# iKrishneel/fcn_object_detector

Measured on AMD Instinct MI355X. Metric: frames/sec forward 448x448 @1 GPU; train imgs/sec @1/2/4/8 GPUs, higher is better.
Workload: dtype f32; 1 GPU; configs[1]: single-GPU forward, DetectNet GoogLeNet conv stack + coverage/bbox heads (graph of models/deploy.prototxt), batch=1, 448x448, random-init weights; global_batch=1, parallelism=replicas x1, frames_in_flight=4

## Files before the change

fcn_object_detector_amd/engine.py:

```python
from __future__ import annotations

import ctypes as C
import os
import threading
from collections import namedtuple
from dataclasses import dataclass, field
from typing import Callable, Dict, List, Optional, Sequence, Tuple, Union

import numpy as np

from . import lib as L
from . import storage as S
from . import tune as T
from .netspec import Layer, NetSpec, bn_global_stats, crop_window, kernel_stride_pad
from .storage import _r4, _ra, ip_pack_bank, ip_unpack_bank

F32 = np.float32


def graphs_enabled() -> bool:
    return os.environ.get("FCN_NO_GRAPH", "0") in ("", "0")


_replica_ctx = threading.local()
# ... 234 lines not shown
        self.score_acc: Dict[str, DeviceBuffer] = {}
        self.graph_score: Optional[int] = None
        if dtype == "f16" and spec.phase != "TEST":
            raise NotImplementedError("the half-float path is inference only (BASELINE configs[4])")
        self.dtype, self.f16 = dtype, dtype == "f16"
        self.spec = spec
        self.device = device
        self.fuse = fuse
        self.group_convs = group_convs
        self.autotune = autotune
        L.call("fcn_init", device)
        sp = C.c_void_p()
        self.replica = replica if replica is not None else _take_replica_index()
        if self.replica is None:
            L.call("fcn_stream_create", C.byref(sp))
        else:
            L.call("fcn_stream_create_replica", C.byref(sp), int(self.replica))
        self.stream = int(sp.value)
        yes = C.c_int(0)
        L.call("fcn_stream_is_prioritized", self.stream, C.byref(yes))
        self.stream_prioritized = bool(yes.value)
        self.lock = threading.RLock()
        self.shapes = spec.infer(data_shapes)
        self.blobs: Dict[str, Blob] = {}
        self.params_host: Dict[str, List[np.ndarray]] = {}
        self.params_dev: Dict[str, List[DevView]] = {}
        self.ops: List[Op] = []
        self.graph_io: Optional[int] = None
        self.graph_core: Optional[int] = None
        self._staging: Dict[str, DeviceBuffer] = {}
        self._keep: List[object] = []
        self._conv_layer_meta: Dict[str, dict] = {}
        self._group_workspaces: List[DeviceBuffer] = []
        self.aux_dev: Dict[str, DeviceBuffer] = {}
        self._bn_chains: Dict[str, BnChain] = {}
        self._bn_ws_bytes = 0
        self._bn_ws: Optional[DeviceBuffer] = None
        self._lazy_blob_ops: Dict[str, List[Op]] = {}
        self.loss_blobs: Dict[str, float] = {}
        self.device_fed: set = set()
        self.dropout_seed = 0
        self.dropout_index_offset = 0
        self.inputs = spec.data_tops()
        self.outputs = [b for b in spec.output_blobs() if b in self.shapes]
        max_lds = int(tune_max_lds_kb if tune_max_lds_kb is not None else os.environ.get("FCN_TUNE_MAX_LDS_KB", "160")) * 1024
        self.tuner = T.Tuner(self.stream, T.key_suffix(self.shapes.get(self.inputs[0], ()) if self.inputs else None, self.f16, max_lds),
                             spec.phase == "TEST", max_lds, tune_from._chosen_cfgs if tune_from is not None else None)
        self._plan_buffers()
        self._alloc_params(params)
        self._build_ops()
        self.tuner.release()

    @property
    def _chosen_cfgs(self) -> Dict[str, object]:
        return self.tuner.chosen

    def _plan_buffers(self) -> None:
        plan = S.plan_blobs(self.spec, self.shapes, self.inputs, self.outputs, self.f16, self.fuse, os.environ.get("FCN_F16_IMAGE", "1") != "0")
        self.producers, self.consumers = plan.producers, plan.consumers
        self.alias, self.shift, self.copy_concats, self.copy_slices = plan.alias, plan.shift, plan.copy_concats, plan.copy_slices
        self._half_inputs = plan.half_inputs
        bufs = {root: DeviceBuffer(nbytes) for root, nbytes in plan.root_bytes.items()}
        for name, v in plan.views.items():
            b = self.blobs[name] = Blob(name, v.shape)
            b.esize, b.rows, b.is_input = v.esize, v.rows, name in self.inputs
            b.buf, b.coffset, b.cstride = bufs[v.root], v.coffset, v.cstride
# ... 27 lines not shown
        for l in self.spec.param_layers():
            if l.name in self.shared_layers:
                continue
            shapes = self.spec.param_shapes[l.name]
            blobs = params.get(l.name)
            if blobs is None:
                raise KeyError("no parameters for layer %s" % l.name)
            host = []
            for arr, shp in zip(blobs, shapes):
                a = np.ascontiguousarray(arr, dtype=F32)
                if a.shape != tuple(shp):
                    if a.size != int(np.prod(shp)):
                        raise ValueError("layer %s: parameter shape %s does not match %s" % (l.name, a.shape, shp))
                    a = a.reshape(shp)
                host.append(a.copy())
            self.params_host[l.name] = host
        self.param_flat = DeviceBuffer(max(self.param_count, 4) * 4, zero=True)
        for seg in self.param_layout:
            self.param_segs[(seg.layer, seg.index)] = seg
            self.params_dev.setdefault(seg.layer, []).append(DevView(self.param_flat.ptr + 4 * seg.offset, seg.nbytes))
        for l in self.spec.param_layers():
            if l.name not in self.shared_layers:
                self._upload_params(l)

    def _folded_shift(self, l: Layer) -> float:
        return next((sh for t, sh in self._half_inputs.values() if t == l.bottoms[0]), 0.0) if l.type == "Convolution" else 0.0

    def _upload_params(self, l: Layer) -> None:
        if l.name in self.shared_layers:
            raise RuntimeError("layer %s reads the parameters of another engine (share_params): set them there" % l.name)
        packed = [S.pack(self.param_segs[(l.name, i)], h, self._folded_shift(l) if i == 0 else 0.0) for i, h in enumerate(self.params_host[l.name])]
        for arr, dev in zip(packed, self.params_dev[l.name]):
            L.call("fcn_memcpy_h2d_async", dev.ptr, arr.ctypes.data, arr.nbytes, None)
        L.call("fcn_device_sync")

    def set_params(self, layer: str, blobs: Sequence[np.ndarray]) -> None:
        lay = next(l for l in self.spec.layers if l.name == layer)
        if layer in self.shared_layers:
            raise RuntimeError("layer %s reads the parameters of another engine (share_params): set them there" % layer)
        shapes = self.spec.param_shapes[layer]
        self.params_host[layer] = [np.ascontiguousarray(b, dtype=F32).reshape(s).copy() for b, s in zip(blobs, shapes)]
        self._upload_params(lay)

    def read_param(self, layer: str, index: int) -> np.ndarray:
        with self.lock:
            v = self.params_dev[layer][index]
            raw = np.empty(v.nbytes, np.uint8)
            L.call("fcn_memcpy_d2h_async", raw.ctypes.data, v.ptr, raw.nbytes, self.stream)
            L.call("fcn_stream_sync", self.stream)
        return S.unpack(self.param_segs[(layer, index)], raw)

    def _geom(self, l: Layer, ksp: Optional[Tuple[int, int, int]] = None) -> ConvGeom:
        n, cin, h, w = self.blobs[l.bottoms[0]].shape
        _, cout, oh, ow = self.blobs[l.tops[0]].shape
        k, s, pad = ksp or kernel_stride_pad(l.sub("pooling_param" if l.type == "Pooling" else "convolution_param"))
        return ConvGeom(n, cin, h, w, cout, oh, ow, k, s, pad)

    def _conv_groups(self, l: Layer) -> int:
        return int(l.sub("convolution_param").get("group", 1)) if l.type == "Convolution" else 1

    def _conv_desc(self, l: Layer, fused_relu: bool, sig_top: Optional[str], group: int = 0) -> L.ConvDesc:
        g, ng = self._geom(l), self._conv_groups(l)
        xb, yb = self.blobs[l.bottoms[0]], self.blobs[l.tops[0]]
        eps = 16 // xb.esize
        if xb.coffset % eps or xb.cstride % eps:
            raise NotImplementedError("conv input view of %s is not 16-byte aligned" % l.name)
# ... 163 lines not shown
            if t == "InnerProduct":
                relu = self._relu_after(li, l, skip)
                self._conv_layer_meta[l.name] = dict(relu=relu, sigmoid_top=None)
                tasks.append(OpTask(l, self._fwd_inner_product(l, relu), reads=[self._range(l.bottoms[0])], writes=[self._range(l.tops[0])]))
                continue
            if t in ("BatchNorm", "Scale"):
                ch = self._bn_chain_after(li, l, skip)
                tasks.append(OpTask(l, self._fwd_batchnorm(ch), reads=[self._range(ch.x)], writes=[self._range(ch.y)]))
                continue
            if t == "Concat" and l.name not in self.copy_concats:
                continue
            if t == "Slice" and l.name not in self.copy_slices:
                continue
            if t == "Dropout" and spec.phase == "TEST" and (l.tops[0] == l.bottoms[0] or l.tops[0] in self.alias):
                continue
            if t == "Power" and l.tops[0] in self.shift:
                continue
            ops = self._emit_simple(l)
            read = l.bottoms[:1] if t == "Crop" else l.bottoms
            tasks.append(OpTask(l, ops, reads=[self._range(b) for b in read], writes=[self._range(tp) for tp in l.tops],
                                pool_desc=self._fusable_pool_desc(l)))
        return tasks

    def _build_ops(self) -> None:
        tasks = self._collect_tasks()
        if self._bn_ws_bytes:
            self._bn_ws = DeviceBuffer(self._bn_ws_bytes, zero=False)
        if self.fuse and self.spec.phase == "TEST" and os.environ.get("FCN_FUSE_POOL_LRN", "1") != "0":
            tasks = self._fuse_pool_lrn(tasks)
        levels = task_levels(tasks, self.group_convs)
        if self.autotune and self.group_convs and self.fuse and not self.f16 and self.spec.phase == "TEST" and os.environ.get("FCN_LEVEL_MOVE", "1") != "0":
            self.tuner.move_floaters(tasks, levels)
        tail = self._plan_tail(tasks, levels)
        order = sorted(range(len(tasks)), key=lambda i: (levels[i], 1 if isinstance(tasks[i], ConvTask) else 0, i))
        pending: List[ConvTask] = []
        pending_pools: List[OpTask] = []
        cur = None
        for i in order:
            if levels[i] != cur:
                self._emit_convs(pending, pending_pools, tail)
                pending, cur = [], levels[i]
            if tail is not None and any(tasks[i] is ht for ht in tail["heads"]):
                continue
            if isinstance(tasks[i], ConvTask):
                pending.append(tasks[i])
            elif tasks[i].pool_desc is not None and self.fuse and self.group_convs:
                pending_pools.append(tasks[i])
            else:
                self.ops.extend(tasks[i].ops)
        self._emit_convs(pending, pending_pools, tail)
        self.levels = max(levels) + 1 if levels else 0
        if self.score_outputs:
            self._emit_score_ops()

    def _emit_group(self, chunk: List[ConvTask], fused: List[OpTask], tail: Optional[dict]) -> None:
        lib = L.load()
        name = "+".join(it.layer.name for it in chunk)
        flops = sum(it.flops for it in chunk)
        byts = sum(it.bytes for it in chunk)
        arr = (L.ConvDesc * len(chunk))(*[it.desc for it in chunk])
        ws = DeviceBuffer(int(lib.fcn_conv2d_group_workspace_bytes(len(chunk))), zero=False)
        self._group_workspaces.append(ws)
        grp = L.ConvGroup()
        parr = (L.PoolDesc * max(len(fused), 1))(*[pt.pool_desc for pt in fused])
        tune_key = name + ("{+%d pool}" % len(fused) if fused else "")
        tailed = tail is not None and any(id(it) in tail["producers"] for it in chunk)
        if tailed:
            fin = 1 if any(tail["producers"][id(it)] == tail["final_level"] for it in chunk if id(it) in tail["producers"]) else 0
            tail["desc"].finalize = fin
            L.call("fcn_conv2d_group_attach_tail", ws.ptr, C.byref(tail["desc"]))
            tune_key += "{+tail%d}" % fin
            if fin:
                flops += sum(ht.flops for ht in tail["heads"])
                byts += sum(4.0 * ht.desc.Cout * (ht.desc.N * ht.desc.OH * ht.desc.OW + ht.desc.Cin) for ht in tail["heads"])
        cfg = self.tuner.conv_cfg(tune_key, arr, len(chunk), ws, parr, len(fused)) if self.autotune else -1
        L.call("fcn_conv2d_group_prepare_fused", arr, len(chunk), parr, len(fused), ws.ptr, cfg, C.byref(grp))
        self._keep.extend([arr, parr, ws, grp])
        kind = "conv_group" if len(chunk) > 1 else "conv"
        label = "%s [cfg%d %dwg]" % (name, grp.cfg, grp.total_tiles)
        if fused:
            label = "%s {+%s}" % (label, "+".join(pt.layer.name for pt in fused))
            byts += sum(pt.ops[0].bytes for pt in fused)
        if tailed:
            label = "%s {%s %s}" % (label, "tail:" if tail["desc"].finalize else "partial sums of", "+".join(ht.layer.name for ht in tail["heads"]))
        self.ops.append(Op(kind, label, lambda st, g=grp: L.check(lib.fcn_conv2d_fwd_group_f32(C.byref(g), st)), flops, byts))

    def _emit_convs(self, items: List[ConvTask], pools: List[OpTask], tail: Optional[dict]) -> None:
        for base in range(0, len(items), 16):
            chunk = items[base:base + 16]
            fused = pools[:2] if base == 0 and len(chunk) <= 8 else []
            parts = [chunk]
            if self.f16 and self.autotune and not fused and len(chunk) > 1:
                parts = self.tuner.split_level(chunk)
            for part in parts:
                self._emit_group(part, fused, tail)
                fused = []
            if base == 0 and len(chunk) <= 8:
                del pools[:2]
        for pt in pools:
            self.ops.extend(pt.ops)
        pools.clear()

    def _emit_score_ops(self) -> None:
        lib = L.load()
        for nm in self.outputs:
            b = self.blobs[nm]
            if b.esize != 4 or b.lazy_shift:
                raise NotImplementedError("score_outputs: output blob %s is not a plain float32 blob" % nm)
            count = int(np.prod(b.shape)) if b.shape else 1
            acc = DeviceBuffer(max(4 * count, 16), zero=True)
            self.score_acc[nm] = acc
            if b.nchw is not None:
                n, c, h, w = b.nchw
                args = (acc.ptr, b.buf.ptr, n, h * w, c, b.cstride, b.coffset)
            else:
                args = (acc.ptr, b.ptr, 1, 1, count, count, 0)
            self.ops.append(Op("score", "score:" + nm, lambda st, a=args: L.check(lib.fcn_score_accumulate_f32(*a, st)), 0.0, 12.0 * count))

    def _plan_tail(self, tasks: List[Task], levels: List[int]) -> Optional[dict]:
        if self.f16 or self.spec.phase != "TEST" or not (self.fuse and self.group_convs) or os.environ.get("FCN_CONV_TAIL", "0") != "1":
            return None
        conv_idx = [i for i, t in enumerate(tasks) if isinstance(t, ConvTask)]
        if not conv_idx:
            return None
        lh = max(levels[i] for i in conv_idx)
        heads = [i for i in conv_idx if levels[i] == lh]
        if any(levels[i] >= lh for i, t in enumerate(tasks) if not isinstance(t, ConvTask)) or not 1 <= len(heads) <= 4:
            return None
        d0 = tasks[heads[0]].desc
        m = d0.N * d0.OH * d0.OW
        rows = 0
        for i in heads:
            d = tasks[i].desc
            if (d.kh, d.kw, d.stride, d.pad) != (1, 1, 1, 0) or d.x != d0.x or d.x_cstride != d0.x_cstride or d.Cin != d0.Cin or d.Cin % 32 or d.Cin > 1024 or d.Cout % 4 \
# ... 800 lines not shown
            for i, op in enumerate(self.ops):
                acc = []
                for _ in range(reps):
                    for prev in self.ops[:i]:
                        prev.run(self.stream)
                    L.call("fcn_event_record", e0, self.stream)
                    op.run(self.stream)
                    L.call("fcn_event_record", e1, self.stream)
                    L.call("fcn_event_sync", e1)
                    L.call("fcn_event_elapsed_ms", e0, e1, C.byref(ms))
                    acc.append(ms.value)
                out.append((op.kind, op.name, float(np.median(acc)), op.flops, op.bytes))
            L.call("fcn_event_destroy", e0)
            L.call("fcn_event_destroy", e1)
        self.event_pair_floor_ms = floor
        return out

    def close(self) -> None:
        with self.lock:
            lib = L.load()
            for g in (self.graph_io, self.graph_core, self.graph_score):
                if g:
                    lib.fcn_graph_destroy(g)
            self.graph_io = self.graph_core = self.graph_score = None
            if self.stream:
                lib.fcn_stream_sync(self.stream)
                lib.fcn_stream_destroy(self.stream)
                self.stream = 0
            for ws in getattr(self, "_group_workspaces", []):
                if ws.ptr:
                    lib.fcn_conv2d_group_release(ws.ptr)
                    ws.free()
            self._group_workspaces = []
            self.ops = []
            self.tuner.release()

    def __del__(self):
        try:
            self.close()
        except Exception:
            pass


class ForwardPipeline:

    def __init__(self, make_spec: Callable[[], NetSpec], params: Optional[Dict[str, List[np.ndarray]]] = None, device: int = 0, depth: int = 4,
                 max_lds_kb: Optional[int] = 36, **engine_kw):
        if depth < 1:
            raise ValueError("depth must be at least 1")
        self.engines: List[Engine] = []
        if os.environ.get("FCN_PIPE_LDS_KB"):
            max_lds_kb = int(os.environ["FCN_PIPE_LDS_KB"]) or None
        if max_lds_kb is not None:
            engine_kw.setdefault("tune_max_lds_kb", max_lds_kb)
        for i in range(depth):
            self.engines.append(Engine(make_spec(), params=params, device=device, tune_from=self.engines[0] if i else None, replica=i,
                                       **engine_kw))
        self._pending: List[Engine] = []
        self._next = 0

    @property
    def depth(self) -> int:
        return len(self.engines)

    def submit(self, inputs: Dict[str, np.ndarray]) -> None:
        if len(self._pending) >= len(self.engines):
# ... 82 lines not shown
```

fcn_object_detector_amd/lib.py:

```python
from __future__ import annotations

import ctypes as C
import os
import threading
from typing import Optional

_HERE = os.path.dirname(os.path.abspath(__file__))
LIB_PATH = os.environ.get("FCN_LIB_PATH") or os.path.join(_HERE, "libfcnhip.so")


class FcnLibraryError(RuntimeError):
    pass


class FcnError(RuntimeError):
    def __init__(self, code: int, msg: str):
        super().__init__("libfcnhip error %d: %s" % (code, msg))
        self.code = code


class ConvDesc(C.Structure):
    _fields_ = [
        ("x", C.c_void_p), ("w", C.c_void_p), ("bias", C.c_void_p), ("y", C.c_void_p), ("y2", C.c_void_p),
        ("N", C.c_int32), ("H", C.c_int32), ("W", C.c_int32), ("Cin", C.c_int32), ("x_cstride", C.c_int32),
# ... 95 lines not shown
    "fcn_memcpy_h2d_async": (_i, [_vp, _vp, _sz, _vp]),
    "fcn_memcpy_d2h_async": (_i, [_vp, _vp, _sz, _vp]),
    "fcn_memcpy_d2d_async": (_i, [_vp, _vp, _sz, _vp]),
    "fcn_stream_create": (_i, [C.POINTER(_vp)]),
    "fcn_stream_destroy": (_i, [_vp]),
    "fcn_stream_sync": (_i, [_vp]),
    "fcn_event_create": (_i, [C.POINTER(_vp)]),
    "fcn_event_destroy": (_i, [_vp]),
    "fcn_event_record": (_i, [_vp, _vp]),
    "fcn_event_sync": (_i, [_vp]),
    "fcn_event_elapsed_ms": (_i, [_vp, _vp, C.POINTER(_f)]),
    "fcn_graph_begin": (_i, [_vp]),
    "fcn_graph_end": (_i, [_vp, C.POINTER(_vp)]),
    "fcn_graph_launch": (_i, [_vp, _vp]),
    "fcn_graph_destroy": (_i, [_vp]),
    "fcn_stream_create_replica": (_i, [C.POINTER(_vp), _i]),
    "fcn_stream_is_prioritized": (_i, [_vp, C.POINTER(_i)]),
    "fcn_nchw_to_nhwc_f32": (_i, [_vp, _vp, _i, _i, _i, _i, _i, _i, _f, _vp]),
    "fcn_nhwc_to_nchw_f32": (_i, [_vp, _vp, _i, _i, _i, _i, _i, _i, _vp]),
    "fcn_nhwc_to_nchw_multi_f32": (_i, [C.POINTER(LayoutDesc), _i, _vp]),
    "fcn_conv2d_fwd_f32": (_i, [C.POINTER(ConvDesc), _vp]),
    "fcn_conv2d_group_workspace_bytes": (_sz, [_i]),
    "fcn_conv2d_num_configs": (_i, []),
    "fcn_conv2d_first_layer_config": (_i, []),
    "fcn_conv2d_config_lds_bytes": (_i, [_i]),
    "fcn_conv2d_config_waves_k": (_i, [_i]),
    "fcn_conv2d_group_prepare": (_i, [C.POINTER(ConvDesc), _i, _vp, _i, C.POINTER(ConvGroup)]),
    "fcn_conv2d_group_prepare_fused": (_i, [C.POINTER(ConvDesc), _i, C.POINTER(PoolDesc), _i, _vp, _i, C.POINTER(ConvGroup)]),
    "fcn_conv2d_fwd_group_f32": (_i, [C.POINTER(ConvGroup), _vp]),
    "fcn_conv2d_group_release": (_i, [_vp]),
    "fcn_conv2d_tail_scratch_bytes": (C.c_size_t, [C.POINTER(ConvTail)]),
    "fcn_conv2d_tail_arrive_bytes": (C.c_size_t, [C.POINTER(ConvTail)]),
    "fcn_conv2d_group_attach_tail": (_i, [_vp, C.POINTER(ConvTail)]),
    "fcn_maxpool_fwd_f32": (_i, [_vp, _vp, _vp] + [_i] * 12 + [_vp]),
    "fcn_avepool_fwd_f32": (_i, [_vp, _vp] + [_i] * 12 + [_vp]),
    "fcn_lrn_fwd_f32": (_i, [_vp, _vp, _vp, _i, _i, _i, _i, _i, _f, _f, _f, _vp]),
    "fcn_maxpool_lrn5_fwd_f32": (_i, [_vp, _vp] + [_i] * 12 + [_f, _f, _f, _vp]),
    "fcn_maxpool_lrn5_fwd_f16": (_i, [_vp, _vp] + [_i] * 12 + [_f, _f, _f, _vp]),
    "fcn_maxpool_lrn5_conv1x1_fwd_f32": (_i, [_vp] + [_i] * 10 + [_f, _f, _f, _vp, _vp, _i, _i, _vp, _i, _i, _vp]),
    "fcn_maxpool_lrn5_conv1x1_fwd_f16": (_i, [_vp] + [_i] * 10 + [_f, _f, _f, _vp, _vp, _i, _i, _vp, _i, _i, _vp]),
    "fcn_relu_fwd_f32": (_i, [_vp, _vp, _sz, _f, _vp]),
    "fcn_sigmoid_fwd_f32": (_i, [_vp, _vp, _sz, _vp]),
    "fcn_power_fwd_f32": (_i, [_vp, _vp, _sz, _f, _f, _f, _vp]),
    "fcn_eltwise_fwd_f32": (_i, [_vp, _vp, _vp, _sz, _i, _f, _f, _vp]),
    "fcn_copy_channels_f32": (_i, [_vp, _vp, _i, _i, _i, _i, _i, _i, _vp]),
    "fcn_deconv_depthwise_fwd_f32": (_i, [_vp, _vp, _vp, _vp] + [_i] * 12 + [_vp]),
    "fcn_preprocess_bgr8": (_i, [_vp, _i, _i, _vp, _i, _i, _i, _f, _vp, _vp]),
    "fcn_detect_workspace_bytes": (_sz, [C.POINTER(DetectParams), _i]),
    "fcn_detect_decode_group": (_i, [_vp, _vp, _i, _sz, _sz, C.POINTER(DetectParams), _vp, _vp, _vp, _vp, _vp]),
    "fcn_score_masks_workspace_bytes": (_sz, [_i, _i, _i, _i]),
    "fcn_score_masks": (_i, [_vp, _i, _i, _i, _i, _i, _i, _vp, _f, _vp, _i, _i, _vp, _vp, _vp]),
    "fcn_gen_targets": (_i, [_vp, _vp, _vp, _i, _i, _i, _i, _i, _d, _vp, _vp, _vp, _vp, _vp, _vp]),
    "fcn_gen_targets_nhwc": (_i, [_vp, _vp, _vp, _i, _i, _i, _i, _i, _d, _vp, _i, _vp, _vp, _vp, _vp, _i, _vp]),
    "fcn_conv2d_wgrad_workspace_floats": (_sz, [C.POINTER(ConvDesc), C.POINTER(_i)]),
    "fcn_conv2d_wgrad_f32": (_i, [C.POINTER(ConvDesc), _vp, _vp, _vp, _vp]),
    "fcn_conv2d_wgrad_group_workspace_floats": (_sz, [C.POINTER(ConvDesc), _i]),
    "fcn_conv2d_wgrad_group_f32": (_i, [C.POINTER(ConvDesc), _vp, _vp, _i, _vp, _vp]),
    "fcn_conv2d_wgrad_num_configs": (_i, []),
    "fcn_conv2d_wgrad_split_config": (_i, []),
    "fcn_conv2d_wgrad_workspace_floats_cfg": (_sz, [C.POINTER(ConvDesc), _i, C.POINTER(_i)]),
    "fcn_conv2d_wgrad_cfg_f32": (_i, [C.POINTER(ConvDesc), _vp, _vp, _vp, _i, _vp]),
    "fcn_conv2d_wgrad_group_workspace_floats_cfg": (_sz, [C.POINTER(ConvDesc), _i, _i]),
    "fcn_conv2d_wgrad_group_cfg_f32": (_i, [C.POINTER(ConvDesc), _vp, _vp, _i, _vp, _i, _vp]),
    "fcn_conv_weights_flip_f32": (_i, [_vp, _vp, _i, _i, _i, _i, _i, _i, _vp]),
    "fcn_nchw_f32_to_nhwc_f16": (_i, [_vp, _vp, _i, _i, _i, _i, _i, _i, _f, _vp]),
    "fcn_nhwc_f16_to_nchw_f32": (_i, [_vp, _vp, _i, _i, _i, _i, _i, _i, _vp]),
# ... 129 lines not shown
```

fcn_object_detector_amd/tune.py:

```python
from __future__ import annotations

import ctypes as C
import json
import os
from typing import Callable, Dict, Iterable, List, NamedTuple, Optional, Sequence, Tuple

import numpy as np

from . import engine as E
from . import lib as L


def lower_quartile(samples: Sequence[float]) -> float:
    return float(np.percentile(samples, 25))


class Protocol(NamedTuple):
    warm: int
    reps: int
    evict: bool
    samples: int
    stat: Callable[[Sequence[float]], float]
    contenders: int
    margin: float
# ... 164 lines not shown
            op.sel["cfg"] = self.choose(self.key("wgrad:" + "+".join(op.layers)), self._valid_cfg(ncfg),
                                        lambda: self.fastest(range(ncfg), select, lambda: op.run(self.stream), WGRAD)[0])
            op.name += " [cfg%d]" % op.sel["cfg"]

    def split_level(self, chunk: List["E.ConvTask"]) -> List[List["E.ConvTask"]]:
        n = len(chunk)
        if n < 2 or n > 4:
            return [chunk]

        def valid(code) -> bool:
            return isinstance(code, str) and len(code) == n and all(ch.isdigit() and int(ch) < n for ch in code)

        def search() -> str:
            memo: Dict[Tuple[int, ...], float] = {}

            def cost(sub: Tuple[int, ...]) -> float:
                if sub not in memo:
                    memo[sub] = self._subset_ms([chunk[i].desc for i in sub])
                return memo[sub]

            best, best_ms = None, 1e30
            for labels in set_partitions(n):
                ms = sum(cost(tuple(i for i in range(n) if labels[i] == g)) for g in sorted(set(labels)))
                if ms < best_ms - 1e-7:
                    best, best_ms = labels, ms
            return "".join(str(g) for g in best)

        choice = self.choose("cut|" + self.key("+".join(it.layer.name for it in chunk)), valid, search)
        groups: Dict[str, List[E.ConvTask]] = {}
        for it, g in zip(chunk, choice):
            groups.setdefault(g, []).append(it)
        return [groups[g] for g in sorted(groups)]

    def move_floaters(self, tasks: Sequence[object], levels: List[int]) -> None:
        for lv in range(max(levels, default=-1)):
            a_idx, b_idx = ([i for i, t in enumerate(tasks) if levels[i] == l2 and isinstance(t, E.ConvTask)] for l2 in (lv, lv + 1))
            if len(a_idx) < 2 or not b_idx or len(a_idx) > 8:
                continue
            fl = [i for i in a_idx if E.task_floats(tasks, levels, i)]
            if not fl or len(fl) > 3 or len(b_idx) + len(fl) > 8:
                continue

            def valid(code) -> bool:
                return isinstance(code, str) and len(code) == len(fl) and set(code) <= {"0", "1"} and (len(fl) < len(a_idx) or "0" in code)

            def search() -> str:
                pools = {l2: [t.pool_desc for j, t in enumerate(tasks) if levels[j] == l2 and isinstance(t, E.OpTask) and t.pool_desc is not None][:2]
                         for l2 in (lv, lv + 1)}
                memo: Dict[Tuple[int, Tuple[int, ...]], float] = {}

                def cost(l2: int, sub: Tuple[int, ...]) -> float:
                    if (l2, sub) not in memo:
                        memo[(l2, sub)] = min(self._subset_ms([tasks[i].desc for i in sub], pools[l2]) for _ in range(2))
                    return memo[(l2, sub)]

                best, best_ms, base_ms = "0" * len(fl), None, None
                for code in range(1 << len(fl)):
                    moved = [fl[b] for b in range(len(fl)) if code >> b & 1]
                    stay = tuple(i for i in a_idx if i not in moved)
                    if not stay:
                        continue
                    ms = cost(lv, stay) + cost(lv + 1, tuple(b_idx + moved))
                    if code == 0:
                        base_ms = ms
                    if best_ms is None or ms < best_ms:
                        best, best_ms = "".join("1" if code >> b & 1 else "0" for b in range(len(fl))), ms
# ... 10 lines not shown
```

include/fcnhip.h:

```cpp
#ifndef FCNHIP_H_
#define FCNHIP_H_

#include <stddef.h>
#include <stdint.h>

#ifdef __cplusplus
extern "C" {
#endif

#define FCN_ABI_VERSION 1

#define FCN_E_ARG       1
#define FCN_E_ALIGN     2
#define FCN_E_UNSUPPORTED 3
#define FCN_E_STATE     4
#define FCN_E_CAPACITY  5

typedef void* fcn_stream_t;
typedef void* fcn_event_t;
typedef void* fcn_graph_t;
typedef void* fcn_comm_t;

int  fcn_abi_version(void);
const char* fcn_last_error_string(void);
// ... 59 lines not shown
} fcn_conv_desc;
int  fcn_conv2d_fwd_f32(const fcn_conv_desc* h_desc, fcn_stream_t s);
typedef struct fcn_conv_group {
    void*   d_probs;
    int32_t n;
    int32_t cfg;
    int32_t total_tiles;
} fcn_conv_group;
size_t fcn_conv2d_group_workspace_bytes(int n);
int  fcn_conv2d_num_configs(void);
int  fcn_conv2d_first_layer_config(void);
typedef struct fcn_conv_tail {
    int32_t n;
    int32_t finalize;
    fcn_conv_desc heads[4];
    float*  scratch;
    void*   arrive;
} fcn_conv_tail;
size_t fcn_conv2d_tail_scratch_bytes(const fcn_conv_tail* t);
size_t fcn_conv2d_tail_arrive_bytes(const fcn_conv_tail* t);
int  fcn_conv2d_group_attach_tail(void* d_workspace, const fcn_conv_tail* t);
int  fcn_conv2d_config_lds_bytes(int cfg);
int  fcn_conv2d_config_waves_k(int cfg);
int  fcn_conv2d_group_prepare(const fcn_conv_desc* h_descs, int n, void* d_workspace, int cfg_request, fcn_conv_group* h_out);
int  fcn_conv2d_fwd_group_f32(const fcn_conv_group* h_group, fcn_stream_t s);
typedef struct fcn_pool_desc {
    const float* x; float* y; int32_t* idx;
    int32_t N, H, W, C, x_cstride, k, stride, pad, OH, OW, y_cstride, y_coffset;
    int32_t f16;
} fcn_pool_desc;
int  fcn_conv2d_group_prepare_fused(const fcn_conv_desc* h_descs, int n, const fcn_pool_desc* h_pools, int npools, void* d_workspace,
                                    int cfg_request, fcn_conv_group* h_out);
int  fcn_conv2d_group_release(void* d_workspace);

int  fcn_maxpool_fwd_f32(const float* x, float* y, int32_t* idx, int N, int H, int W, int C,
                         int x_cstride, int k, int stride, int pad, int OH, int OW,
                         int y_cstride, int y_coffset, fcn_stream_t s);
int  fcn_avepool_fwd_f32(const float* x, float* y, int N, int H, int W, int C, int x_cstride,
                         int k, int stride, int pad, int OH, int OW, int y_cstride, int y_coffset,
                         fcn_stream_t s);
int  fcn_lrn_fwd_f32(const float* x, float* y, float* scale, int pixels, int C, int x_cstride,
                     int y_cstride, int local_size, float alpha, float beta, float k, fcn_stream_t s);
int  fcn_maxpool_lrn5_fwd_f32(const float* x, float* y, int N, int H, int W, int C, int x_cstride, int k, int stride, int pad,
                              int OH, int OW, int y_cstride, int lrn_first, float alpha, float beta, float lrn_k, fcn_stream_t s);
int  fcn_maxpool_lrn5_conv1x1_fwd_f32(const float* x, int N, int H, int W, int C, int x_cstride, int k, int stride, int pad,
                                      int OH, int OW, float alpha, float beta, float lrn_k, const float* w, const float* bias,
                                      int Cout, int relu, float* y, int y_cstride, int y_coffset, fcn_stream_t s);
int  fcn_maxpool_lrn5_conv1x1_fwd_f16(const void* x, int N, int H, int W, int C, int x_cstride, int k, int stride, int pad,
                                      int OH, int OW, float alpha, float beta, float lrn_k, const void* w, const float* bias,
                                      int Cout, int relu, void* y, int y_cstride, int y_coffset, fcn_stream_t s);
int  fcn_relu_fwd_f32(const float* x, float* y, size_t count, float negative_slope, fcn_stream_t s);
int  fcn_sigmoid_fwd_f32(const float* x, float* y, size_t count, fcn_stream_t s);
int  fcn_power_fwd_f32(const float* x, float* y, size_t count, float power, float scale, float shift, fcn_stream_t s);
#define FCN_ELT_PROD 0
#define FCN_ELT_SUM  1
#define FCN_ELT_MAX  2
int  fcn_eltwise_fwd_f32(const float* a, const float* b, float* y, size_t count, int op,
                         float ca, float cb, fcn_stream_t s);
int  fcn_copy_channels_f32(const float* src, float* dst, int pixels, int C, int src_cstride,
                           int src_coffset, int dst_cstride, int dst_coffset, fcn_stream_t s);
int  fcn_softmax_fwd_f32(const float* x, float* y, int pixels, int C, int x_cstride, int y_cstride, fcn_stream_t s);
int  fcn_deconv_depthwise_fwd_f32(const float* x, const float* w, const float* bias, float* y,
                                  int N, int H, int W, int C, int x_cstride, int k, int stride, int pad,
                                  int OH, int OW, int y_cstride, int y_coffset, fcn_stream_t s);

int  fcn_preprocess_bgr8(const uint8_t* frame, int h, int w, float* dst, int H, int W, int dst_cstride,
// ... 229 lines not shown
```

Measured before the change: 4376 frames/s.

## Add Winograd F(2x2,3x3) conv path with per-level autotuned selection

Adds a Winograd F(2x2,3x3) path for 3x3 stride-1 pad-1 f32 convolutions. Filters are pre-transformed once into a bank; at run time an input-transform kernel runs, then a fused MFMA GEMM kernel whose producer waves stream tiles into LDS and whose consumer waves compute, with the output transform, bias and ReLU in the epilogue. The tuner times each candidate layer on its own against the remaining grouped direct-conv launch and keeps Winograd only when the split is cheaper. The aim is fewer multiplies for the 3x3 convs, at the cost of a workspace round trip through global memory, an extra kernel launch, slightly different rounding, and transformed-filter banks that may go stale if parameters are set later.

```diff
diff --git a/fcn_object_detector_amd/csrc/conv_winograd.hip b/fcn_object_detector_amd/csrc/conv_winograd.hip
--- /dev/null
+++ b/fcn_object_detector_amd/csrc/conv_winograd.hip
@@ -0,0 +1,381 @@
+#include "conv_common.h"
+
+namespace fcn {
+namespace {
+
+struct WinoP {
+    const float* x;
+    const float* U;
+    float* V;
+    const float* bias;
+    float* y;
+    int N, H, W, Cin, x_cstride;
+    int Cout, y_cstride, y_coffset, flags;
+    int TH, TW, tiles, Tpad, Cpad, KC;
+    int tiles_n;
+};
+
+constexpr int kWinoVariants = 2;
+constexpr int kWinoThreads = 512;
+constexpr int kRing = 8;
+
+inline int round_up(int a, int b) { return (a + b - 1) / b * b; }
+
+__global__ __launch_bounds__(256) void wino_filter_kernel(const float* __restrict__ w, float* __restrict__ U, int Cout, int Cin, int Cpad) {
+    const long long gid = (long long)blockIdx.x * 256 + threadIdx.x;
+    if (gid >= (long long)Cout * Cpad) return;
+    const int co = (int)(gid / Cpad), c = (int)(gid % Cpad);
+    double g[3][3];
+#pragma unroll
+    for (int i = 0; i < 3; ++i)
+#pragma unroll
+        for (int j = 0; j < 3; ++j) g[i][j] = c < Cin ? (double)w[((size_t)(co * 3 + i) * 3 + j) * Cin + c] : 0.0;
+    double t[4][3];
+#pragma unroll
+    for (int j = 0; j < 3; ++j) {
+        t[0][j] = g[0][j];
+        t[1][j] = 0.5 * ((g[0][j] + g[1][j]) + g[2][j]);
+        t[2][j] = 0.5 * ((g[0][j] - g[1][j]) + g[2][j]);
+        t[3][j] = g[2][j];
+    }
+    float* u = U + ((size_t)co * 16) * Cpad + c;
+#pragma unroll
+    for (int i = 0; i < 4; ++i) {
+        u[(size_t)(4 * i + 0) * Cpad] = (float)t[i][0];
+        u[(size_t)(4 * i + 1) * Cpad] = (float)(0.5 * ((t[i][0] + t[i][1]) + t[i][2]));
+        u[(size_t)(4 * i + 2) * Cpad] = (float)(0.5 * ((t[i][0] - t[i][1]) + t[i][2]));
+        u[(size_t)(4 * i + 3) * Cpad] = (float)t[i][2];
+    }
+}
+
+__global__ __launch_bounds__(256) void wino_input_kernel(const WinoP p) {
+    const int cq = p.Cpad >> 2;
+    const long long gid = (long long)blockIdx.x * 256 + threadIdx.x;
+    if (gid >= (long long)p.Tpad * cq) return;
+    const int tile = (int)(gid / cq), c = (int)(gid % cq) * 4;
+    v4f d[4][4];
+#pragma unroll
+    for (int i = 0; i < 4; ++i)
+#pragma unroll
+        for (int j = 0; j < 4; ++j) d[i][j] = v4f{0.f, 0.f, 0.f, 0.f};
+    if (tile < p.tiles && c < p.Cin) {
+        const int tx = tile % p.TW, t2 = tile / p.TW, ty = t2 % p.TH, img = t2 / p.TH;
+#pragma unroll
+        for (int i = 0; i < 4; ++i) {
+            const int iy = 2 * ty - 1 + i;
+#pragma unroll
+            for (int j = 0; j < 4; ++j) {
+                const int ix = 2 * tx - 1 + j;
+                if ((unsigned)iy < (unsigned)p.H && (unsigned)ix < (unsigned)p.W)
+                    d[i][j] = *(const v4f*)(p.x + ((size_t)(img * p.H + iy) * p.W + ix) * p.x_cstride + c);
+            }
+        }
+    }
+    v4f t[4][4];
+#pragma unroll
+    for (int j = 0; j < 4; ++j) {
+        t[0][j] = d[0][j] - d[2][j];
+        t[1][j] = d[1][j] + d[2][j];
+        t[2][j] = d[2][j] - d[1][j];
+        t[3][j] = d[1][j] - d[3][j];
+    }
+    const size_t plane = (size_t)p.Tpad * p.Cpad;
+    float* v = p.V + (size_t)tile * p.Cpad + c;
+#pragma unroll
+    for (int i = 0; i < 4; ++i) {
+        *(v4f*)(v + (size_t)(4 * i + 0) * plane) = t[i][0] - t[i][2];
+        *(v4f*)(v + (size_t)(4 * i + 1) * plane) = t[i][1] + t[i][2];
+        *(v4f*)(v + (size_t)(4 * i + 2) * plane) = t[i][2] - t[i][1];
+        *(v4f*)(v + (size_t)(4 * i + 3) * plane) = t[i][1] - t[i][3];
+    }
+}
+
+template <int TM>
+struct WinoCfg {
+    static constexpr int A_FLOATS = 32 * 32;
+    static constexpr int B_FLOATS = TM * 32;
+    static constexpr int SLOT_FLOATS = A_FLOATS + B_FLOATS;
+    static constexpr int LDS_FLOATS = kRing * SLOT_FLOATS;
+    static constexpr int IA = 4, IB = TM / 8;
+};
+
+template <int TM>
+__global__ __launch_bounds__(kWinoThreads, 2) void wino_fused_kernel(const WinoP p) {
+    using C = WinoCfg<TM>;
+    __shared__ __attribute__((aligned(1024))) float smem[C::LDS_FLOATS];
+    const int tid = threadIdx.x, lane = tid & 63;
+    const int wave = __builtin_amdgcn_readfirstlane(tid >> 6);
+    const int tile_m = (int)blockIdx.x / p.tiles_n, tile_n = (int)blockIdx.x - tile_m * p.tiles_n;
+    const int co0 = tile_n * 32, t0 = tile_m * TM;
+    const int G = 4 * p.KC;
+
+    if (wave >= 4) {
+        const int w = wave - 4;
+        constexpr int OOB = (int)0x80000000u;
+        const __amdgpu_buffer_rsrc_t ru = __builtin_amdgcn_make_buffer_rsrc(const_cast<float*>(p.U), 0, p.Cout * 16 * p.Cpad * 4, 0x00020000);
+        const __amdgpu_buffer_rsrc_t rv = __builtin_amdgcn_make_buffer_rsrc(p.V, 0, 16 * p.Tpad * p.Cpad * 4, 0x00020000);
+        int a_vo[C::IA], b_vo[C::IB];
+#pragma unroll
+        for (int i = 0; i < C::IA; ++i) {
+            const int row = 8 * i + (lane >> 3), seg = (lane & 7) ^ swz<8>(row), co = co0 + row;
+            a_vo[i] = co < p.Cout ? (co * 16 * p.Cpad + seg * 4) * 4 : OOB;
+        }
+#pragma unroll
+        for (int i = 0; i < C::IB; ++i) {
+            const int row = 8 * i + (lane >> 3), seg = (lane & 7) ^ swz<8>(row);
+            b_vo[i] = ((t0 + row) * p.Cpad + seg * 4) * 4;
+        }
+        const int u_tap = p.Cpad * 4, v_plane = p.Tpad * p.Cpad * 4;
+        auto issue_group = [&](const int g) {
+            const int j = g & 3, kc = g >> 2, t = 4 * w + j;
+            float* dst = smem + ((g & 1) * 4 + w) * C::SLOT_FLOATS;
+            const int s_a = t * u_tap + kc * 128, s_b = t * v_plane + kc * 128;
+#if defined(__HIP_DEVICE_COMPILE__)
+#pragma unroll
+            for (int i = 0; i < C::IA; ++i) __builtin_amdgcn_raw_ptr_buffer_load_lds(ru, (lds_ptr)(dst + 256 * i), 16, a_vo[i], s_a, 0, 0);
+#pragma unroll
+            for (int i = 0; i < C::IB; ++i)
+                __builtin_amdgcn_raw_ptr_buffer_load_lds(rv, (lds_ptr)(dst + C::A_FLOATS + 256 * i), 16, b_vo[i], s_b, 0, 0);
+#else
+            (void)dst, (void)s_a, (void)s_b, (void)ru, (void)rv;
+#endif
+        };
+        issue_group(0);
+#pragma unroll 1
+        for (int g = 0; g < G; ++g) {
+            wait_vmcnt<0>();
+            __builtin_amdgcn_s_barrier();
+            asm volatile("" ::: "memory");
+            if (g + 1 < G) issue_group(g + 1);
+        }
+        __builtin_amdgcn_s_barrier();
+        asm volatile("" ::: "memory");
+    } else {
+        const int r = wave;
+        if constexpr (TM == 32) {
+            f32x16 acc[4];
+#pragma unroll
+            for (int j = 0; j < 4; ++j)
+#pragma unroll
+                for (int q = 0; q < 16; ++q) acc[j][q] = 0.f;
+            const int row = lane & 31, fs = swz<8>(row);
+            int fo[4];
+#pragma unroll
+            for (int st = 0; st < 4; ++st) fo[st] = r * C::SLOT_FLOATS + row * 32 + (((2 * st + (lane >> 5)) ^ fs) << 2);
+#pragma unroll 1
+            for (int g0 = 0; g0 < G; g0 += 4) {
+#pragma unroll
+                for (int j = 0; j < 4; ++j) {
+                    asm volatile("s_waitcnt lgkmcnt(0)" ::: "memory");
+                    __builtin_amdgcn_s_barrier();
+                    asm volatile("" ::: "memory");
+                    const float* slot = smem + (j & 1) * 4 * C::SLOT_FLOATS;
+                    v4f a[4], b[4];
+#pragma unroll
+                    for (int st = 0; st < 4; ++st) {
+                        a[st] = *(const v4f*)(slot + fo[st]);
+                        b[st] = *(const v4f*)(slot + C::A_FLOATS + fo[st]);
+                    }
+                    __builtin_amdgcn_sched_barrier(0);
+#pragma unroll
+                    for (int st = 0; st < 4; ++st)
+#pragma unroll
+                        for (int e = 0; e < 4; ++e) acc[j] = __builtin_amdgcn_mfma_f32_32x32x2f32(a[st][e], b[st][e], acc[j], 0, 0, 0);
+                }
+            }
+            asm volatile("s_waitcnt lgkmcnt(0)" ::: "memory");
+            __builtin_amdgcn_s_barrier();
+            asm volatile("" ::: "memory");
+#pragma unroll
+            for (int q = 0; q < 4; ++q) {
+                v4f p0, p1;
+#pragma unroll
+                for (int e = 0; e < 4; ++e) {
+                    const int k = 4 * q + e;
+                    p0[e] = (acc[0][k] + acc[1][k]) + acc[2][k];
+                    p1[e] = (acc[1][k] - acc[2][k]) - acc[3][k];
+                }
+                const int ch = 8 * q + 4 * (lane >> 5);
+                *(v4f*)(smem + ((2 * r + 0) * TM + row) * 32 + ch) = p0;
+                *(v4f*)(smem + ((2 * r + 1) * TM + row) * 32 + ch) = p1;
+            }
+        } else {
+            v4f acc[4][2];
+#pragma unroll
+            for (int j = 0; j < 4; ++j)
+#pragma unroll
+                for (int h = 0; h < 2; ++h) acc[j][h] = v4f{0.f, 0.f, 0.f, 0.f};
+            const int row = lane & 15;
+            int fa[2][2], fb[2];
+#pragma unroll
+            for (int st = 0; st < 2; ++st) {
+                const int seg = 4 * st + (lane >> 4);
+                fa[0][st] = r * C::SLOT_FLOATS + row * 32 + ((seg ^ swz<8>(row)) << 2);
+                fa[1][st] = r * C::SLOT_FLOATS + (row + 16) * 32 + ((seg ^ swz<8>(row + 16)) << 2);
+                fb[st] = r * C::SLOT_FLOATS + C::A_FLOATS + row * 32 + ((seg ^ swz<8>(row)) << 2);
+            }
+#pragma unroll 1
+            for (int g0 = 0; g0 < G; g0 += 4) {
+#pragma unroll
+                for (int j = 0; j < 4; ++j) {
+                    asm volatile("s_waitcnt lgkmcnt(0)" ::: "memory");
+                    __builtin_amdgcn_s_barrier();
+                    asm volatile("" ::: "memory");
+                    const float* slot = smem + (j & 1) * 4 * C::SLOT_FLOATS;
+                    v4f a[2][2], b[2];
+#pragma unroll
+                    for (int st = 0; st < 2; ++st) {
+                        a[0][st] = *(const v4f*)(slot + fa[0][st]);
+                        a[1][st] = *(const v4f*)(slot + fa[1][st]);
+                        b[st] = *(const v4f*)(slot + fb[st]);
+                    }
+                    __builtin_amdgcn_sched_barrier(0);
+#pragma unroll
+                    for (int st = 0; st < 2; ++st)
+#pragma unroll
+                        for (int e = 0; e < 4; ++e)
+#pragma unroll
+                            for (int h = 0; h < 2; ++h)
+                                acc[j][h] = __builtin_amdgcn_mfma_f32_16x16x4f32(a[h][st][e], b[st][e], acc[j][h], 0, 0, 0);
+                }
+            }
+            asm volatile("s_waitcnt lgkmcnt(0)" ::: "memory");
+            __builtin_amdgcn_s_barrier();
+            asm volatile("" ::: "memory");
+#pragma unroll
+            for (int h = 0; h < 2; ++h) {
+                const v4f p0 = (acc[0][h] + acc[1][h]) + acc[2][h];
+                const v4f p1 = (acc[1][h] - acc[2][h]) - acc[3][h];
+                const int ch = 16 * h + 4 * (lane >> 4);
+                *(v4f*)(smem + ((2 * r + 0) * TM + row) * 32 + ch) = p0;
+                *(v4f*)(smem + ((2 * r + 1) * TM + row) * 32 + ch) = p1;
+            }
+        }
+    }
+    __syncthreads();
+
+#pragma unroll
+    for (int item = tid; item < TM * 32; item += kWinoThreads) {
+        const int cq = item & 7, jj = (item >> 3) & 1, i = (item >> 4) & 1, tl = item >> 5;
+        const int gt = t0 + tl;
+        if (gt >= p.tiles) continue;
+        const int tx = gt % p.TW, t2 = gt / p.TW, ty = t2 % p.TH, img = t2 / p.TH;
+        const int oy = 2 * ty + i, ox = 2 * tx + jj, ch = co0 + 4 * cq;
+        if (oy >= p.H || ox >= p.W || ch >= p.Cout) continue;
+        v4f P[4];
+#pragma unroll
+        for (int rr = 0; rr < 4; ++rr) P[rr] = *(const v4f*)(smem + ((2 * rr + jj) * TM + tl) * 32 + 4 * cq);
+        v4f yv = i == 0 ? (P[0] + P[1]) + P[2] : (P[1] - P[2]) - P[3];
+        if (p.bias) {
+#pragma unroll
+            for (int e = 0; e < 4; ++e) yv[e] += p.bias[ch + e < p.Cout ? ch + e : p.Cout - 1];
+        }
+        if (p.flags & FCN_CONV_RELU) {
+#pragma unroll
+            for (int e = 0; e < 4; ++e) yv[e] = fmaxf(yv[e], 0.f);
+        }
+        float* dst = p.y + ((size_t)(img * p.H + oy) * p.W + ox) * p.y_cstride + p.y_coffset + ch;
+        if (ch + 4 <= p.Cout) {
+            *(v4f*)dst = yv;
+        } else {
+#pragma unroll
+            for (int e = 0; e < 4; ++e)
+                if (ch + e < p.Cout) dst[e] = yv[e];
+        }
+    }
+}
+
+int wino_check(const fcn_conv_desc* d, bool need_ptrs) {
+    FCN_REQUIRE(d != nullptr, FCN_E_ARG, "winograd: null descriptor");
+    FCN_REQUIRE(d->N > 0 && d->H > 0 && d->W > 0 && d->Cin > 0 && d->Cout > 0, FCN_E_ARG, "winograd: non-positive extent");
+    FCN_REQUIRE(d->kh == 3 && d->kw == 3 && d->stride == 1 && d->pad == 1, FCN_E_UNSUPPORTED,
+                "winograd: only 3x3 / stride 1 / pad 1 (got %dx%d stride %d pad %d)", d->kh, d->kw, d->stride, d->pad);
+    FCN_REQUIRE(d->OH == d->H && d->OW == d->W, FCN_E_ARG, "winograd: OH x OW must equal H x W");
+    FCN_REQUIRE((d->flags & ~FCN_CONV_RELU) == 0, FCN_E_UNSUPPORTED, "winograd: only bias and FCN_CONV_RELU (flags 0x%x)", d->flags);
+    FCN_REQUIRE(d->in_shift == 0.f, FCN_E_UNSUPPORTED, "winograd: in_shift must be 0");
+    FCN_REQUIRE(d->Cin % 4 == 0, FCN_E_UNSUPPORTED, "winograd: Cin %d is not a multiple of 4", d->Cin);
+    FCN_REQUIRE(d->x_cstride >= d->Cin && d->y_cstride >= d->y_coffset + d->Cout && d->y_coffset >= 0, FCN_E_ARG,
+                "winograd: slice wider than its stride");
+    FCN_REQUIRE(d->x_cstride % 4 == 0 && d->y_cstride % 4 == 0 && d->y_coffset % 4 == 0, FCN_E_ALIGN,
+                "winograd: strides and offsets must be multiples of 4 floats");
+    const long long tiles = (long long)d->N * ((d->H + 1) / 2) * ((d->W + 1) / 2), tpad = (tiles + 31) / 32 * 32;
+    const long long cpad = (d->Cin + 31) / 32 * 32;
+    FCN_REQUIRE(16 * tpad * cpad * 4 < (1ll << 31) && (long long)d->Cout * 16 * cpad * 4 < (1ll << 31) &&
+                    (long long)d->N * d->H * d->W * d->x_cstride < (1ll << 31) && (long long)d->N * d->H * d->W * d->y_cstride < (1ll << 31),
+                FCN_E_UNSUPPORTED, "winograd: a tensor past 2^31 bytes / elements");
+    if (need_ptrs) {
+        FCN_REQUIRE(d->x && d->w && d->y, FCN_E_ARG, "winograd: null pointer");
+        FCN_REQUIRE(((uintptr_t)d->x | (uintptr_t)d->y | (uintptr_t)d->w) % 16 == 0, FCN_E_ALIGN, "winograd: x, w and y must be 16-byte aligned");
+    }
+    return 0;
+}
+
+WinoP make_params(const fcn_conv_desc* d, const float* U, float* V) {
+    WinoP p{};
+    p.x = d->x, p.U = U, p.V = V, p.bias = d->bias, p.y = d->y;
+    p.N = d->N, p.H = d->H, p.W = d->W, p.Cin = d->Cin, p.x_cstride = d->x_cstride;
+    p.Cout = d->Cout, p.y_cstride = d->y_cstride, p.y_coffset = d->y_coffset, p.flags = d->flags;
+    p.TH = (d->H + 1) / 2, p.TW = (d->W + 1) / 2;
+    p.tiles = d->N * p.TH * p.TW, p.Tpad = round_up(p.tiles, 32);
+    p.Cpad = round_up(d->Cin, 32), p.KC = p.Cpad / 32;
+    p.tiles_n = (d->Cout + 31) / 32;
+    return p;
+}
+
+}
+}
+
+using namespace fcn;
+
+extern "C" {
+
+int fcn_winograd_num_variants(void) { return kWinoVariants; }
+
+int fcn_winograd_ok(const fcn_conv_desc* h_desc) { return wino_check(h_desc, false); }
+
+int fcn_winograd_variant_lds_bytes(int variant) {
+    return variant == 0 ? WinoCfg<32>::LDS_FLOATS * 4 : variant == 1 ? WinoCfg<16>::LDS_FLOATS * 4 : -1;
+}
+
+size_t fcn_winograd_workspace_bytes(const fcn_conv_desc* h_desc) {
+    if (wino_check(h_desc, false)) return 0;
+    const WinoP p = make_params(h_desc, nullptr, nullptr);
+    return (size_t)16 * p.Tpad * p.Cpad * 4;
+}
+
+size_t fcn_winograd_filter_bytes(const fcn_conv_desc* h_desc) {
+    if (wino_check(h_desc, false)) return 0;
+    return (size_t)h_desc->Cout * 16 * round_up(h_desc->Cin, 32) * 4;
+}
+
+int fcn_winograd_transform_filters(const fcn_conv_desc* h_desc, float* U, fcn_stream_t s) {
+    if (int rc = wino_check(h_desc, false)) return rc;
+    FCN_REQUIRE(h_desc->w && U, FCN_E_ARG, "winograd: null pointer");
+    FCN_REQUIRE(((uintptr_t)h_desc->w | (uintptr_t)U) % 16 == 0, FCN_E_ALIGN, "winograd: w and U must be 16-byte aligned");
+    const int cpad = round_up(h_desc->Cin, 32);
+    const long long n = (long long)h_desc->Cout * cpad;
+    hipLaunchKernelGGL(wino_filter_kernel, dim3(cdiv(n, 256)), dim3(256), 0, as_stream(s), h_desc->w, U, h_desc->Cout, h_desc->Cin, cpad);
+    FCN_LAUNCH_CHECK("wino_filter_kernel");
+    return 0;
+}
+
+int fcn_winograd_conv3x3_f32(const fcn_conv_desc* h_desc, const float* U, float* V_workspace, int variant, fcn_stream_t s) {
+    if (int rc = wino_check(h_desc, true)) return rc;
+    FCN_REQUIRE(U && V_workspace, FCN_E_ARG, "winograd: null pointer");
+    FCN_REQUIRE(((uintptr_t)U | (uintptr_t)V_workspace) % 16 == 0, FCN_E_ALIGN, "winograd: U and the workspace must be 16-byte aligned");
+    FCN_REQUIRE(variant >= -1 && variant < kWinoVariants, FCN_E_ARG, "winograd: unknown variant %d", variant);
+    const WinoP p = make_params(h_desc, U, V_workspace);
+    if (variant < 0) variant = (p.Tpad / 32) * p.tiles_n >= 256 ? 0 : 1;
+    const long long items = (long long)p.Tpad * (p.Cpad / 4);
+    hipLaunchKernelGGL(wino_input_kernel, dim3(cdiv(items, 256)), dim3(256), 0, as_stream(s), p);
+    FCN_LAUNCH_CHECK("wino_input_kernel");
+    if (variant == 0) {
+        hipLaunchKernelGGL(wino_fused_kernel<32>, dim3((p.Tpad / 32) * p.tiles_n), dim3(kWinoThreads), 0, as_stream(s), p);
+    } else {
+        hipLaunchKernelGGL(wino_fused_kernel<16>, dim3(cdiv(p.tiles, 16) * p.tiles_n), dim3(kWinoThreads), 0, as_stream(s), p);
+    }
+    FCN_LAUNCH_CHECK("wino_fused_kernel");
+    return 0;
+}
+
+}
diff --git a/fcn_object_detector_amd/engine.py b/fcn_object_detector_amd/engine.py
--- a/fcn_object_detector_amd/engine.py
+++ b/fcn_object_detector_amd/engine.py
@@ -290,6 +290,9 @@
         self._keep: List[object] = []
         self._conv_layer_meta: Dict[str, dict] = {}
         self._group_workspaces: List[DeviceBuffer] = []
+        self._wino_mode = os.environ.get("FCN_CONV_WINOGRAD", "") or "0"
+        self._wino_banks: Dict[str, Tuple[L.ConvDesc, DeviceBuffer]] = {}
+        self._wino_scratch: Optional[DeviceBuffer] = None
         self.aux_dev: Dict[str, DeviceBuffer] = {}
         self._bn_chains: Dict[str, BnChain] = {}
         self._bn_ws_bytes = 0
@@ -383,6 +386,10 @@
         packed = [S.pack(self.param_segs[(l.name, i)], h, self._folded_shift(l) if i == 0 else 0.0) for i, h in enumerate(self.params_host[l.name])]
         for arr, dev in zip(packed, self.params_dev[l.name]):
             L.call("fcn_memcpy_h2d_async", dev.ptr, arr.ctypes.data, arr.nbytes, None)
+        wino = getattr(self, "_wino_banks", {}).get(l.name)
+        if wino is not None:
+            d, bank = wino
+            L.call("fcn_winograd_transform_filters", C.byref(d), bank.ptr, None)
         L.call("fcn_device_sync")
 
     def set_params(self, layer: str, blobs: Sequence[np.ndarray]) -> None:
@@ -612,6 +619,7 @@
         if self.autotune and self.group_convs and self.fuse and not self.f16 and self.spec.phase == "TEST" and os.environ.get("FCN_LEVEL_MOVE", "1") != "0":
             self.tuner.move_floaters(tasks, levels)
         tail = self._plan_tail(tasks, levels)
+        self._all_conv_tasks = [t for t in tasks if isinstance(t, ConvTask)]
         order = sorted(range(len(tasks)), key=lambda i: (levels[i], 1 if isinstance(tasks[i], ConvTask) else 0, i))
         pending: List[ConvTask] = []
         pending_pools: List[OpTask] = []
@@ -666,6 +674,14 @@
         self.ops.append(Op(kind, label, lambda st, g=grp: L.check(lib.fcn_conv2d_fwd_group_f32(C.byref(g), st)), flops, byts))
 
     def _emit_convs(self, items: List[ConvTask], pools: List[OpTask], tail: Optional[dict]) -> None:
+        wino = self._winograd_pick(items, pools, tail)
+        if wino:
+            items = [it for it in items if all(it is not w for w, _ in wino)]
+        self._emit_direct(items, pools, tail)
+        for it, variant in wino:
+            self._emit_winograd(it, variant)
+
+    def _emit_direct(self, items: List[ConvTask], pools: List[OpTask], tail: Optional[dict]) -> None:
         for base in range(0, len(items), 16):
             chunk = items[base:base + 16]
             fused = pools[:2] if base == 0 and len(chunk) <= 8 else []
@@ -680,6 +696,61 @@
         for pt in pools:
             self.ops.extend(pt.ops)
         pools.clear()
+
+    def _winograd_bank(self, it: ConvTask) -> DeviceBuffer:
+        lib = L.load()
+        name = it.layer.name
+        if name not in self._wino_banks:
+            bank = DeviceBuffer(int(lib.fcn_winograd_filter_bytes(C.byref(it.desc))), zero=False)
+            L.call("fcn_winograd_transform_filters", C.byref(it.desc), bank.ptr, None)
+            L.call("fcn_device_sync")
+            self._wino_banks[name] = (it.desc, bank)
+        assert int(lib.fcn_winograd_workspace_bytes(C.byref(it.desc))) <= self._wino_scratch.nbytes
+        return self._wino_banks[name][1]
+
+    def _winograd_candidates(self, items: List[ConvTask], tail: Optional[dict]) -> List[ConvTask]:
+        mode = getattr(self, "_wino_mode", "0")
+        if mode == "0" or self.f16 or self.spec.phase != "TEST" or self._share_from is not None:
+            return []
+        if mode != "1" and not self.autotune:
+            return []
+        lib = L.load()
+        return [it for it in items if self._conv_groups(it.layer) == 1 and lib.fcn_winograd_ok(C.byref(it.desc)) == 0
+                and not (tail is not None and id(it) in tail["producers"])]
+
+    def _winograd_pick(self, items: List[ConvTask], pools: List[OpTask], tail: Optional[dict]) -> List[Tuple[ConvTask, int]]:
+        cand = self._winograd_candidates(items, tail)
+        if not cand:
+            return []
+        if self._wino_scratch is None:
+            lib = L.load()
+            every = [t for t in self._all_conv_tasks if lib.fcn_winograd_ok(C.byref(t.desc)) == 0]
+            self._wino_scratch = DeviceBuffer(max(int(lib.fcn_winograd_workspace_bytes(C.byref(t.desc))) for t in every), zero=False)
+        if self._wino_mode == "1":
+            picked = [(it, -1) for it in cand]
+        else:
+            code = self.tuner.winograd_level(items, pools[:2] if len(items) <= 8 else [], cand, self._winograd_launcher)
+            picked = [(it, int(ch)) for it, ch in zip(cand, code) if ch != "-"]
+        for it in cand:
+            if all(it is not p for p, _ in picked) and it.layer.name in self._wino_banks:
+                self._wino_banks.pop(it.layer.name)[1].free()
+        for it, _ in picked:
+            self._winograd_bank(it)
+        return picked
+
+    def _winograd_launcher(self, it: ConvTask) -> Callable[[int, Optional[int]], None]:
+        lib = L.load()
+        bank, d = self._winograd_bank(it), it.desc
+        return lambda variant, st: L.check(lib.fcn_winograd_conv3x3_f32(C.byref(d), bank.ptr, self._wino_scratch.ptr, variant, st))
+
+    def _emit_winograd(self, it: ConvTask, variant: int) -> None:
+        launch = self._winograd_launcher(it)
+        d = it.desc
+        tiles = d.N * ((d.H + 1) // 2) * ((d.W + 1) // 2)
+        v_bytes = 2.0 * 16 * tiles * ((d.Cin + 31) // 32 * 32) * 4
+        label = "%s [winograd F(2x2,3x3) v%s: input transform + fused GEMM, flops = direct conv]" % (it.layer.name, variant if variant >= 0 else "auto")
+        self._keep.append(d)
+        self.ops.append(Op("conv_winograd", label, lambda st, v=variant: launch(v, st), it.flops, it.bytes + v_bytes))
 
     def _emit_score_ops(self) -> None:
         lib = L.load()
@@ -1546,6 +1617,12 @@
                     lib.fcn_conv2d_group_release(ws.ptr)
                     ws.free()
             self._group_workspaces = []
+            for _, bank in getattr(self, "_wino_banks", {}).values():
+                bank.free()
+            self._wino_banks = {}
+            if getattr(self, "_wino_scratch", None) is not None:
+                self._wino_scratch.free()
+                self._wino_scratch = None
             self.ops = []
             self.tuner.release()
 
diff --git a/fcn_object_detector_amd/lib.py b/fcn_object_detector_amd/lib.py
--- a/fcn_object_detector_amd/lib.py
+++ b/fcn_object_detector_amd/lib.py
@@ -151,6 +151,13 @@
     "fcn_conv2d_tail_scratch_bytes": (C.c_size_t, [C.POINTER(ConvTail)]),
     "fcn_conv2d_tail_arrive_bytes": (C.c_size_t, [C.POINTER(ConvTail)]),
     "fcn_conv2d_group_attach_tail": (_i, [_vp, C.POINTER(ConvTail)]),
+    "fcn_winograd_num_variants": (_i, []),
+    "fcn_winograd_variant_lds_bytes": (_i, [_i]),
+    "fcn_winograd_ok": (_i, [C.POINTER(ConvDesc)]),
+    "fcn_winograd_workspace_bytes": (_sz, [C.POINTER(ConvDesc)]),
+    "fcn_winograd_filter_bytes": (_sz, [C.POINTER(ConvDesc)]),
+    "fcn_winograd_transform_filters": (_i, [C.POINTER(ConvDesc), _vp, _vp]),
+    "fcn_winograd_conv3x3_f32": (_i, [C.POINTER(ConvDesc), _vp, _vp, _i, _vp]),
     "fcn_maxpool_fwd_f32": (_i, [_vp, _vp, _vp] + [_i] * 12 + [_vp]),
     "fcn_avepool_fwd_f32": (_i, [_vp, _vp] + [_i] * 12 + [_vp]),
     "fcn_lrn_fwd_f32": (_i, [_vp, _vp, _vp, _i, _i, _i, _i, _i, _f, _f, _f, _vp]),
diff --git a/fcn_object_detector_amd/tune.py b/fcn_object_detector_amd/tune.py
--- a/fcn_object_detector_amd/tune.py
+++ b/fcn_object_detector_amd/tune.py
@@ -220,6 +220,43 @@
             groups.setdefault(g, []).append(it)
         return [groups[g] for g in sorted(groups)]
 
+    def winograd_level(self, chunk: List["E.ConvTask"], pools: Sequence["E.OpTask"], cand: List["E.ConvTask"],
+                       launcher: Callable[["E.ConvTask"], Callable[[int, Optional[int]], None]]) -> str:
+        nvar = int(L.load().fcn_winograd_num_variants())
+        cold = self.cold and os.environ.get("FCN_TUNE_COLD", "1") != "0"
+        pdescs = [pt.pool_desc for pt in pools]
+
+        def valid(code) -> bool:
+            return isinstance(code, str) and len(code) == len(cand) and all(ch == "-" or (ch.isdigit() and int(ch) < nvar) for ch in code)
+
+        def search() -> str:
+            state = list(chunk)
+            cur_ms = min(self._subset_ms([t.desc for t in state], pdescs) for _ in range(2))
+            code = []
+            for it in cand:
+                rest = [t for t in state if t is not it]
+                if not rest and pdescs:
+                    code.append("-")
+                    continue
+                launch = launcher(it)
+                sel = {"v": 0}
+
+                def select(v: int) -> bool:
+                    sel["v"] = v
+                    return True
+
+                v, pair_ms = self.fastest(range(nvar), select, lambda: launch(sel["v"], self.stream), COLD if cold else WARM)
+                rest_ms = min(self._subset_ms([t.desc for t in rest], pdescs) for _ in range(2)) if rest else 0.0
+                if pair_ms + rest_ms <= float(os.environ.get("FCN_MOVE_MARGIN", "0.99")) * cur_ms:
+                    state, cur_ms = rest, pair_ms + rest_ms
+                    code.append(str(v))
+                else:
+                    code.append("-")
+            return "".join(code)
+
+        name = "+".join(t.layer.name for t in chunk) + ("{+%d pool}" % len(pdescs) if pdescs else "")
+        return self.choose("wino|" + self.key(name), valid, search)
+
     def move_floaters(self, tasks: Sequence[object], levels: List[int]) -> None:
         for lv in range(max(levels, default=-1)):
             a_idx, b_idx = ([i for i, t in enumerate(tasks) if levels[i] == l2 and isinstance(t, E.ConvTask)] for l2 in (lv, lv + 1))
diff --git a/include/fcnhip.h b/include/fcnhip.h
--- a/include/fcnhip.h
+++ b/include/fcnhip.h
@@ -115,6 +115,14 @@
 int  fcn_conv2d_group_prepare_fused(const fcn_conv_desc* h_descs, int n, const fcn_pool_desc* h_pools, int npools, void* d_workspace,
                                     int cfg_request, fcn_conv_group* h_out);
 int  fcn_conv2d_group_release(void* d_workspace);
+
+int    fcn_winograd_num_variants(void);
+int    fcn_winograd_variant_lds_bytes(int variant);
+int    fcn_winograd_ok(const fcn_conv_desc* h_desc);
+size_t fcn_winograd_workspace_bytes(const fcn_conv_desc* h_desc);
+size_t fcn_winograd_filter_bytes(const fcn_conv_desc* h_desc);
+int    fcn_winograd_transform_filters(const fcn_conv_desc* h_desc, float* U, fcn_stream_t s);
+int    fcn_winograd_conv3x3_f32(const fcn_conv_desc* h_desc, const float* U, float* V_workspace, int variant, fcn_stream_t s);
 
 int  fcn_maxpool_fwd_f32(const float* x, float* y, int32_t* idx, int N, int H, int W, int C,
                          int x_cstride, int k, int stride, int pad, int OH, int OW,
```

Result: slower. 3962 frames/s (-9.5%).
